# PRBonn/LiDiff

Hardware: NVIDIA H100
Metric: denoising_steps_per_sec_180k_pts_T50 (higher is better)
Workload: dtype fp16x3 split tensor-core MMA, fp32 accumulate (fp32 CUDA cores for the Cin=3 stem), fp64 DPM update

## Files before the change

### lidiff_b200/csrc/spconv_tc.cu

```cuda
#include "common.cuh"
#include <algorithm>
#include <stdlib.h>
#include "tc_common.cuh"

namespace tc {

constexpr int THREADS = 384;
constexpr int NUM_PRODUCER = 128;
constexpr int NUM_CONSUMER_WARPS = 8;
constexpr int STEP_BUDGET = 64;
constexpr int MAX_KVOL = 27;
constexpr int MAX_STAGES = 4;

struct Params {
    int c1, c2, cout, kvol;
    const unsigned char* wpacked;
    const float* scale;
    const float* shift;
    int relu;
    const int* nbr;
    long long nbr_stride;
    const int* d_mout;
    int mout_cap;
    const int* row_perm;
    const unsigned* row_mask;
    const int* tile_order;
    int stages, nchunks, group;
    int npass, nsplit;
    lb2_conv_io io[2];
};

constexpr int PRODUCER_REGS = 88;
constexpr int CONSUMER_REGS = 208;
static_assert(128 * PRODUCER_REGS + 256 * CONSUMER_REGS <= THREADS * 168, "register split exceeds the CTA's allocation");

template <int NC>
__global__ void __launch_bounds__(THREADS, 1) k_spconv_tc(const Params p) {
    extern __shared__ unsigned char smem_raw[];
    const int M = p.d_mout ? min(*p.d_mout, p.mout_cap) : p.mout_cap;
    const int half = blockIdx.x % p.nsplit;
    const int pass = (blockIdx.x / p.nsplit) % p.npass;
    const int slot_i = blockIdx.x / (p.nsplit * p.npass);
    const int tile = p.tile_order ? __ldg(p.tile_order + slot_i) : slot_i;
    const int m0 = tile * BM;
    if (tile < 0 || m0 >= M) return;
    const lb2_conv_io io = p.io[pass];
    const int n0 = half * NC;
    const int warp = threadIdx.x >> 5, lane = threadIdx.x & 31;
    const int ctot = p.c1 + p.c2;

    const uint32_t raw = smem_u32(smem_raw);
    const uint32_t base = (raw + 1023u) & ~1023u;
    unsigned char* gen = smem_raw + (base - raw);
    constexpr uint32_t b_tile = (uint32_t)NC * 128u;
    const uint32_t b_full = (uint32_t)p.cout * 128u;
    const uint32_t stage_bytes = 2u * A_TILE + 2u * b_tile;
    unsigned char* tail = gen + (size_t)p.stages * stage_bytes;
    int* idx_s = reinterpret_cast<int*>(tail);
    uint64_t* bars = reinterpret_cast<uint64_t*>(tail + MAX_KVOL * BM * sizeof(int));
    uint32_t* misc = reinterpret_cast<uint32_t*>(bars + 3 * MAX_STAGES);
    int* row_s = reinterpret_cast<int*>(misc + 4);
    const uint32_t bar0 = smem_u32(bars);
    auto full_a = [&](int s) { return bar0 + 8u * s; };
    auto full_b = [&](int s) { return bar0 + 8u * (MAX_STAGES + s); };
    auto empty = [&](int s) { return bar0 + 8u * (2 * MAX_STAGES + s); };

    if (threadIdx.x == 0) {
        for (int s = 0; s < p.stages; ++s) { mbar_init(full_a(s), NUM_PRODUCER); mbar_init(full_b(s), 1); mbar_init(empty(s), NUM_CONSUMER_WARPS); }
        misc[1] = 0;
        asm volatile("fence.mbarrier_init.release.cluster;" ::: "memory");
    }
    __syncthreads();
    if (threadIdx.x < BM) {
        const int slot = m0 + threadIdx.x;
        const int row = (slot < M) ? (p.row_perm ? __ldg(p.row_perm + slot) : slot) : -1;
        row_s[threadIdx.x] = row;
        const uint32_t want = row < 0 ? 0u : (p.row_mask ? __ldg(p.row_mask + row) : ~0u);
        int v[MAX_KVOL];
#pragma unroll
        for (int k = 0; k < MAX_KVOL; ++k) {
            v[k] = -1;
            if (k < p.kvol && ((want >> k) & 1u)) v[k] = p.nbr ? __ldg(p.nbr + (long long)k * p.nbr_stride + row) : row;
        }
        uint32_t have = 0;
#pragma unroll
        for (int k = 0; k < MAX_KVOL; ++k) {
            if (k < p.kvol) {
                idx_s[k * BM + threadIdx.x] = v[k];
                if (v[k] >= 0) have |= 1u << k;
            }
        }
        const uint32_t mymask = __reduce_or_sync(0xffffffffu, have);
        if (lane == 0 && mymask) atomicOr(&misc[1], mymask);
    }
    __syncthreads();
    const uint32_t kmask = misc[1];
    const int n_off = __popc(kmask);

    if (warpgroup_role() == 0) {
        setmaxnreg_dec<PRODUCER_REGS>();
        const int sub = threadIdx.x & 7;
        const int rbase = threadIdx.x >> 3;
        const bool use_h = (io.in1_h != nullptr) && (p.c2 == 0 || io.in2_h != nullptr);
        const int D = max(p.stages - 2, 0);
        int it = 0, arrived = 0;
        for (uint32_t km = kmask; km; km &= km - 1) {
            const int k = __ffs(km) - 1;
            const int* idxk = idx_s + k * BM;
            int src[8];
#pragma unroll
            for (int j = 0; j < 8; ++j) src[j] = idxk[rbase + 16 * j];
            for (int c = 0; c < p.nchunks; ++c, ++it) {
                const int s = it % p.stages;
                mbar_wait(empty(s), ((it / p.stages) & 1) ^ 1);
                unsigned char* a_hi = gen + (size_t)s * stage_bytes;
                const uint32_t a_hi_u = base + (uint32_t)s * stage_bytes;
                if (threadIdx.x == 0) {
                    const uint32_t dst = a_hi_u + 2u * A_TILE;
                    const unsigned char* wsrc = p.wpacked + PACK_HEADER + ((size_t)k * p.nchunks + c) * (2u * b_full) + (size_t)n0 * 128u;
                    mbar_expect_tx(full_b(s), 2u * b_tile);
                    bulk_g2s(dst, wsrc, b_tile, full_b(s));
                    bulk_g2s(dst + b_tile, wsrc + b_full, b_tile, full_b(s));
                }
                const int ch = c * KC + sub * 8;
                if (ch < ctot) {
                    const bool first = ch < p.c1;
                    const int cw = first ? p.c1 : p.c2;
                    const int co = first ? ch : ch - p.c1;
                    if (use_h) produce_a_split(reinterpret_cast<const __half*>(first ? io.in1_h : io.in2_h), cw, co, src, a_hi_u, a_hi_u + A_TILE, rbase, sub);
                    else produce_a_f32(first ? io.in1 : io.in2, cw, co, src, a_hi, a_hi + A_TILE, rbase, sub);
                }
                if (use_h) {
                    cp_async_commit();
                    if (it >= D) {
                        cp_async_wait_dyn(D);
                        fence_proxy_async();
                        mbar_arrive(full_a(arrived % p.stages));
                        ++arrived;
                    }
                } else {
                    fence_proxy_async();
                    mbar_arrive(full_a(s));
                }
            }
        }
        if (use_h) {
            cp_async_wait<0>();
            fence_proxy_async();
            for (; arrived < it; ++arrived) mbar_arrive(full_a(arrived % p.stages));
        }
    } else {
        setmaxnreg_inc<CONSUMER_REGS>();
        const int wg = (warp >> 2) - 1;
        float acc[NC / 2], tot[NC / 2];
#pragma unroll
        for (int i = 0; i < NC / 2; ++i) tot[i] = -0.f;
        const int n_it = n_off * p.nchunks;
        int c = 0, in_group = 0, off_idx = 0, prev_s = -1;
        for (int it = 0; it < n_it; ++it) {
            const int s = it % p.stages;
            const uint32_t par = (it / p.stages) & 1;
            mbar_wait(full_b(s), par);
            mbar_wait(full_a(s), par);
            const uint32_t a_hi = base + (uint32_t)s * stage_bytes + (uint32_t)wg * (A_TILE / 2), a_lo = a_hi + A_TILE;
            const uint32_t b_hi = base + (uint32_t)s * stage_bytes + 2u * A_TILE, b_lo = b_hi + b_tile;
            const int ksteps = min(KC, ctot - c * KC) >> 4;
            reg_fence(acc);
            wg_stage_mma<NC>(acc, a_hi, a_lo, b_hi, b_lo, ksteps, in_group == 0 && c == 0);
            reg_fence(acc);
            wgmma_wait<1>();
            if (prev_s >= 0 && lane == 0) mbar_arrive(empty(prev_s));
            prev_s = s;
            if (++c < p.nchunks) continue;
            c = 0;
            ++off_idx;
            if (++in_group == p.group || off_idx == n_off) {
                wgmma_wait<0>();
                reg_fence(acc);
                if (lane == 0) mbar_arrive(empty(prev_s));
                prev_s = -1;
#pragma unroll
                for (int i = 0; i < NC / 2; ++i) tot[i] = __fadd_rn(tot[i], acc[i]);
                in_group = 0;
            }
        }
        wgmma_wait<0>();
        const float out_scale = __ldg(reinterpret_cast<const float*>(p.wpacked) + 1);
        float* stage_c = reinterpret_cast<float*>(gen);
        constexpr int pitch = NC + 4;
        asm volatile("bar.sync 1, 256;" ::: "memory");
        {
            const int r0 = wg * 64 + (warp & 3) * 16 + (lane >> 2);
#pragma unroll
            for (int i = 0; i < NC / 2; i += 2) {
                const int row = r0 + 8 * ((i >> 1) & 1), col = 8 * (i >> 2) + 2 * (lane & 3);
                *reinterpret_cast<float2*>(stage_c + row * pitch + col) = make_float2(tot[i] * out_scale, tot[i + 1] * out_scale);
            }
        }
        asm volatile("bar.sync 1, 256;" ::: "memory");
        const int cw = warp - 4;
        constexpr int nv = NC >> 2;
        for (int e = lane; e < (BM / NUM_CONSUMER_WARPS) * nv; e += 32) {
            const int rr = cw + NUM_CONSUMER_WARPS * (e / nv);
            const int lcol = (e % nv) * 4;
            const int col = n0 + lcol;
            const int orow = row_s[rr];
            if (orow < 0) continue;
            const long long ro = (long long)orow * p.cout;
            const float4 a4 = *reinterpret_cast<const float4*>(stage_c + (size_t)rr * pitch + lcol);
            float y[4] = {a4.x, a4.y, a4.z, a4.w};
            if (io.pre_add) {
                const float4 t4 = __ldg(reinterpret_cast<const float4*>(io.pre_add + ro + col));
                y[0] += t4.x; y[1] += t4.y; y[2] += t4.z; y[3] += t4.w;
            }
            if (p.scale) {
                const float4 s4 = __ldg(reinterpret_cast<const float4*>(p.scale + col));
                const float4 h4 = __ldg(reinterpret_cast<const float4*>(p.shift + col));
                y[0] = fmaf(y[0], s4.x, h4.x); y[1] = fmaf(y[1], s4.y, h4.y); y[2] = fmaf(y[2], s4.z, h4.z); y[3] = fmaf(y[3], s4.w, h4.w);
            }
            if (io.residual || io.residual_h) {
                const float4 t4 = load_residual4(io.residual, io.residual_h, orow, p.cout, col);
                y[0] += t4.x; y[1] += t4.y; y[2] += t4.z; y[3] += t4.w;
            }
            if (p.relu) {
#pragma unroll
                for (int j = 0; j < 4; ++j) y[j] = fmaxf(y[j], 0.f);
            }
            if (io.out) *reinterpret_cast<float4*>(io.out + ro + col) = make_float4(y[0], y[1], y[2], y[3]);
            if (io.out_h) store_split4(io.out_h, orow, p.cout, col, y);
            if (io.out_gated || io.out_gated_h) {
                if (io.gate_table) {
                    const long long g = io.gate_idx ? __ldg(io.gate_idx + orow) : 0;
                    const float4 g4 = __ldg(reinterpret_cast<const float4*>(io.gate_table + g * p.cout + col));
                    y[0] *= g4.x; y[1] *= g4.y; y[2] *= g4.z; y[3] *= g4.w;
                }
                if (io.out_gated) *reinterpret_cast<float4*>(io.out_gated + ro + col) = make_float4(y[0], y[1], y[2], y[3]);
                if (io.out_gated_h) store_split4(io.out_gated_h, orow, p.cout, col, y);
            }
        }
    }
}

__global__ void k_weight_absmax(const float* __restrict__ w, long long n, unsigned* __restrict__ header) {
    long long t = (long long)blockIdx.x * blockDim.x + threadIdx.x;
    float m = 0.f;
    for (; t < n; t += (long long)gridDim.x * blockDim.x) m = fmaxf(m, fabsf(w[t]));
#pragma unroll
    for (int o = 16; o > 0; o >>= 1) m = fmaxf(m, __shfl_xor_sync(0xffffffffu, m, o));
    if ((threadIdx.x & 31) == 0) atomicMax(header, __float_as_uint(m));
}

__device__ __forceinline__ float weight_scale(unsigned max_bits) {
    const float m = __uint_as_float(max_bits);
    if (!(m > 0.f) || !isfinite(m)) return 1.f;
    int e;
    frexpf(m, &e);
    return ldexpf(1.f, 14 - e);
}

__global__ void k_pack_weights(const float* __restrict__ w, int kvol, int cin, int cout, int nchunks, unsigned char* __restrict__ out) {
    const long long total = (long long)kvol * nchunks * cout * KC;
    long long t = (long long)blockIdx.x * blockDim.x + threadIdx.x;
    const float scale = weight_scale(*reinterpret_cast<const unsigned*>(out));
    if (t == 0) reinterpret_cast<float*>(out)[1] = 1.0f / scale;
    if (t >= total) return;
    const int kk = (int)(t % KC);
    const int n = (int)((t / KC) % cout);
    const int c = (int)((t / ((long long)KC * cout)) % nchunks);
    const int k = (int)(t / ((long long)KC * cout * nchunks));
    const int ch = c * KC + kk;
    const float v = ch < cin ? w[((long long)k * cin + ch) * cout + n] * scale : 0.f;
    const __half hi = __float2half_rn(v);
    const __half lo = __float2half_rn(v - __half2float(hi));
    const size_t tile = (size_t)cout * 128;
    unsigned char* blob = out + PACK_HEADER + ((size_t)k * nchunks + c) * 2 * tile;
    const uint32_t off = sw128(n, kk >> 3) + (uint32_t)(kk & 7) * 2u;
    *reinterpret_cast<__half*>(blob + off) = hi;
    *reinterpret_cast<__half*>(blob + tile + off) = lo;
}

static bool shape_ok(int c1, int c2, int cout, int kvol) {
    const int ctot = c1 + c2;
    if (kvol < 1 || kvol > MAX_KVOL) return false;
    if (ctot % 16 != 0 || ctot < 16) return false;
    if (c2 > 0 && (c1 % 8 != 0 || c2 % 8 != 0)) return false;
    if (cout % 32 != 0 || cout < 32 || cout > 256) return false;
    if (cout > 128 && cout != 256) return false;
    return true;
}

static size_t smem_bytes(int nc, int stages) {
    return 1024 + (size_t)stages * (2 * A_TILE + 2 * (size_t)nc * 128) + MAX_KVOL * BM * sizeof(int) + 3 * MAX_STAGES * 8 + 16 + BM * sizeof(int);
}

template <int NC>
static int launch(Lb2Handle* h, cudaStream_t s, const Params& p, int stages) {
    const size_t smem = smem_bytes(NC, stages);
    cudaError_t e = lb2_configure_smem(h, LB2_K_TC + (NC / 32 - 1), k_spconv_tc<NC>, (int)(227 * 1024));
    if (e != cudaSuccess) return lb2_fail(h, LB2_ERR_CUDA, "k_spconv_tc smem attribute: %s", cudaGetErrorString(e));
    k_spconv_tc<NC><<<cdiv(p.mout_cap, BM) * p.npass * p.nsplit, THREADS, smem, s>>>(p);
    LB2_POST_LAUNCH(h, "k_spconv_tc");
    return LB2_OK;
}

}

bool lb2_spconv_tc_supported(const lb2_conv_desc* d) { return tc::shape_ok(d->c1, d->c2, d->cout, d->kvol); }

extern "C" size_t lb2_packed_weight_bytes(int32_t kvol, int32_t cin, int32_t cout) {
    if (!tc::shape_ok(cin, 0, cout, kvol)) return 0;
    const int nchunks = (cin + tc::KC - 1) / tc::KC;
    return tc::PACK_HEADER + (size_t)kvol * nchunks * 2 * (size_t)cout * 128;
}

extern "C" int lb2_pack_weights(void* handle, void* stream, const float* weight, int32_t kvol, int32_t cin, int32_t cout, void* packed) {
    Lb2Handle* h = (Lb2Handle*)handle;
    LB2_REQUIRE(h, h && weight && packed, "pack_weights null");
    if (!tc::shape_ok(cin, 0, cout, kvol)) return lb2_fail(h, LB2_ERR_UNSUP, "pack_weights: shape not supported by the tensor-core variant%s", "");
    const int nchunks = (cin + tc::KC - 1) / tc::KC;
    const long long total = (long long)kvol * nchunks * cout * tc::KC;
    const long long nw = (long long)kvol * cin * cout;
    if (cudaMemsetAsync(packed, 0, tc::PACK_HEADER, (cudaStream_t)stream) != cudaSuccess) return lb2_fail(h, LB2_ERR_CUDA, "pack_weights memset%s", "");
    tc::k_weight_absmax<<<(unsigned)std::min<long long>(cdiv(nw, 256), 1024), 256, 0, (cudaStream_t)stream>>>(weight, nw, (unsigned*)packed);
    LB2_POST_LAUNCH(h, "k_weight_absmax");
    tc::k_pack_weights<<<cdiv(total, 256), 256, 0, (cudaStream_t)stream>>>(weight, kvol, cin, cout, nchunks, (unsigned char*)packed);
    LB2_POST_LAUNCH(h, "k_pack_weights");
    return LB2_OK;
}

int lb2_spconv_tc_launch(Lb2Handle* h, cudaStream_t s, const lb2_conv_desc* d) {
    tc::Params p;
    p.c1 = d->c1; p.c2 = d->c2; p.cout = d->cout; p.kvol = d->kvol;
    p.wpacked = (const unsigned char*)d->weight_packed;
    p.scale = d->scale; p.shift = d->shift; p.relu = d->relu;
    p.nbr = d->nbr; p.nbr_stride = d->nbr_stride; p.d_mout = d->d_mout; p.mout_cap = d->mout_cap; p.row_perm = d->row_perm;
    p.tile_order = d->nbr ? d->tile_order128 : nullptr;
    p.row_mask = d->nbr ? (const unsigned*)d->row_mask : nullptr;
    p.nchunks = (d->c1 + d->c2 + tc::KC - 1) / tc::KC;
    const int nsplit = d->cout > 128 ? 2 : 1;
    const int nc = d->cout / nsplit;
    p.npass = d->npass > 1 ? 2 : 1;
    p.nsplit = nsplit;
    int stages = tc::MAX_STAGES;
    while (stages > 2 && tc::smem_bytes(nc, stages) > 227 * 1024) --stages;
    p.stages = stages;
    const int steps_per_offset = 3 * ((d->c1 + d->c2 + 15) / 16);
    p.group = std::max(1, tc::STEP_BUDGET / steps_per_offset);
    p.io[0] = d->io[0]; p.io[1] = d->io[d->npass > 1 ? 1 : 0];
    switch (nc) {
        case 32: return tc::launch<32>(h, s, p, stages);
        case 64: return tc::launch<64>(h, s, p, stages);
        case 96: return tc::launch<96>(h, s, p, stages);
        case 128: return tc::launch<128>(h, s, p, stages);
        default: return lb2_fail(h, LB2_ERR_UNSUP, "tensor-core variant: no kernel for %s output channels per CTA", nc == 80 ? "80" : nc == 112 ? "112" : "this many");
    }
}
```

Baseline: 25.98.

## Make sparse-conv tensor-core kernel persistent with double-buffered tile metadata

Turns the warp-specialized sparse conv kernel into a persistent kernel with a grid capped at the SM count. Each CTA walks tiles in a grid-stride loop. The producer warpgroup prefetches the next tile's neighbor indices into a double-buffered shared TileInfo, and the epilogue staging reuses a pipeline stage buffer with an XOR swizzle instead of a padded pitch. The aim is to remove per-CTA launch and setup costs and to overlap index loading and the epilogue with the next tile's MMA pipeline. In exchange it adds more complex barrier and parity bookkeeping and an extra pipeline slot per tile, and tile_order load balancing becomes a static round-robin.

After: 27.39 (median of 6 runs). 1.05x the previous value.

```diff
diff --git a/lidiff_b200/csrc/spconv_tc.cu b/lidiff_b200/csrc/spconv_tc.cu
--- a/lidiff_b200/csrc/spconv_tc.cu
+++ b/lidiff_b200/csrc/spconv_tc.cu
@@ -34,20 +34,22 @@
 constexpr int CONSUMER_REGS = 208;
 static_assert(128 * PRODUCER_REGS + 256 * CONSUMER_REGS <= THREADS * 168, "register split exceeds the CTA's allocation");
 
+struct TileInfo {
+    int idx[MAX_KVOL * BM];
+    int row[BM];
+    uint32_t mask[4];
+    int item;
+    int pad[3];
+};
+constexpr int NUM_BARS = 3 * MAX_STAGES + 4;
+
 template <int NC>
 __global__ void __launch_bounds__(THREADS, 1) k_spconv_tc(const Params p) {
     extern __shared__ unsigned char smem_raw[];
     const int M = p.d_mout ? min(*p.d_mout, p.mout_cap) : p.mout_cap;
-    const int half = blockIdx.x % p.nsplit;
-    const int pass = (blockIdx.x / p.nsplit) % p.npass;
-    const int slot_i = blockIdx.x / (p.nsplit * p.npass);
-    const int tile = p.tile_order ? __ldg(p.tile_order + slot_i) : slot_i;
-    const int m0 = tile * BM;
-    if (tile < 0 || m0 >= M) return;
-    const lb2_conv_io io = p.io[pass];
-    const int n0 = half * NC;
     const int warp = threadIdx.x >> 5, lane = threadIdx.x & 31;
     const int ctot = p.c1 + p.c2;
+    const int S = p.stages;
 
     const uint32_t raw = smem_u32(smem_raw);
     const uint32_t base = (raw + 1023u) & ~1023u;
@@ -55,187 +57,229 @@
     constexpr uint32_t b_tile = (uint32_t)NC * 128u;
     const uint32_t b_full = (uint32_t)p.cout * 128u;
     const uint32_t stage_bytes = 2u * A_TILE + 2u * b_tile;
-    unsigned char* tail = gen + (size_t)p.stages * stage_bytes;
-    int* idx_s = reinterpret_cast<int*>(tail);
-    uint64_t* bars = reinterpret_cast<uint64_t*>(tail + MAX_KVOL * BM * sizeof(int));
-    uint32_t* misc = reinterpret_cast<uint32_t*>(bars + 3 * MAX_STAGES);
-    int* row_s = reinterpret_cast<int*>(misc + 4);
-    const uint32_t bar0 = smem_u32(bars);
+    TileInfo* info = reinterpret_cast<TileInfo*>(gen + (size_t)S * stage_bytes);
+    const uint32_t bar0 = smem_u32(info + 2);
     auto full_a = [&](int s) { return bar0 + 8u * s; };
     auto full_b = [&](int s) { return bar0 + 8u * (MAX_STAGES + s); };
     auto empty = [&](int s) { return bar0 + 8u * (2 * MAX_STAGES + s); };
+    auto info_full = [&](int b) { return bar0 + 8u * (3 * MAX_STAGES + b); };
+    auto info_empty = [&](int b) { return bar0 + 8u * (3 * MAX_STAGES + 2 + b); };
 
     if (threadIdx.x == 0) {
-        for (int s = 0; s < p.stages; ++s) { mbar_init(full_a(s), NUM_PRODUCER); mbar_init(full_b(s), 1); mbar_init(empty(s), NUM_CONSUMER_WARPS); }
-        misc[1] = 0;
+        for (int s = 0; s < S; ++s) { mbar_init(full_a(s), NUM_PRODUCER); mbar_init(full_b(s), 1); mbar_init(empty(s), NUM_CONSUMER_WARPS); }
+        for (int b = 0; b < 2; ++b) { mbar_init(info_full(b), NUM_PRODUCER); mbar_init(info_empty(b), NUM_CONSUMER_WARPS); }
         asm volatile("fence.mbarrier_init.release.cluster;" ::: "memory");
     }
     __syncthreads();
-    if (threadIdx.x < BM) {
-        const int slot = m0 + threadIdx.x;
-        const int row = (slot < M) ? (p.row_perm ? __ldg(p.row_perm + slot) : slot) : -1;
-        row_s[threadIdx.x] = row;
-        const uint32_t want = row < 0 ? 0u : (p.row_mask ? __ldg(p.row_mask + row) : ~0u);
-        int v[MAX_KVOL];
-#pragma unroll
-        for (int k = 0; k < MAX_KVOL; ++k) {
-            v[k] = -1;
-            if (k < p.kvol && ((want >> k) & 1u)) v[k] = p.nbr ? __ldg(p.nbr + (long long)k * p.nbr_stride + row) : row;
-        }
-        uint32_t have = 0;
-#pragma unroll
-        for (int k = 0; k < MAX_KVOL; ++k) {
-            if (k < p.kvol) {
-                idx_s[k * BM + threadIdx.x] = v[k];
-                if (v[k] >= 0) have |= 1u << k;
-            }
-        }
-        const uint32_t mymask = __reduce_or_sync(0xffffffffu, have);
-        if (lane == 0 && mymask) atomicOr(&misc[1], mymask);
-    }
-    __syncthreads();
-    const uint32_t kmask = misc[1];
-    const int n_off = __popc(kmask);
 
     if (warpgroup_role() == 0) {
         setmaxnreg_dec<PRODUCER_REGS>();
         const int sub = threadIdx.x & 7;
         const int rbase = threadIdx.x >> 3;
-        const bool use_h = (io.in1_h != nullptr) && (p.c2 == 0 || io.in2_h != nullptr);
-        const int D = max(p.stages - 2, 0);
+        const int D = max(S - 2, 0);
         int it = 0, arrived = 0;
-        for (uint32_t km = kmask; km; km &= km - 1) {
-            const int k = __ffs(km) - 1;
-            const int* idxk = idx_s + k * BM;
-            int src[8];
-#pragma unroll
-            for (int j = 0; j < 8; ++j) src[j] = idxk[rbase + 16 * j];
-            for (int c = 0; c < p.nchunks; ++c, ++it) {
-                const int s = it % p.stages;
-                mbar_wait(empty(s), ((it / p.stages) & 1) ^ 1);
-                unsigned char* a_hi = gen + (size_t)s * stage_bytes;
-                const uint32_t a_hi_u = base + (uint32_t)s * stage_bytes;
-                if (threadIdx.x == 0) {
-                    const uint32_t dst = a_hi_u + 2u * A_TILE;
-                    const unsigned char* wsrc = p.wpacked + PACK_HEADER + ((size_t)k * p.nchunks + c) * (2u * b_full) + (size_t)n0 * 128u;
-                    mbar_expect_tx(full_b(s), 2u * b_tile);
-                    bulk_g2s(dst, wsrc, b_tile, full_b(s));
-                    bulk_g2s(dst + b_tile, wsrc + b_full, b_tile, full_b(s));
-                }
-                const int ch = c * KC + sub * 8;
-                if (ch < ctot) {
-                    const bool first = ch < p.c1;
-                    const int cw = first ? p.c1 : p.c2;
-                    const int co = first ? ch : ch - p.c1;
-                    if (use_h) produce_a_split(reinterpret_cast<const __half*>(first ? io.in1_h : io.in2_h), cw, co, src, a_hi_u, a_hi_u + A_TILE, rbase, sub);
-                    else produce_a_f32(first ? io.in1 : io.in2, cw, co, src, a_hi, a_hi + A_TILE, rbase, sub);
-                }
-                if (use_h) {
+        auto tile_of = [&](int x) {
+            const int slot_i = x / (p.nsplit * p.npass);
+            return slot_i * BM >= p.mout_cap ? -1 : p.tile_order ? __ldg(p.tile_order + slot_i) : slot_i;
+        };
+        auto load_row = [&](int tile) {
+            const int slot = tile * BM + threadIdx.x;
+            return (tile >= 0 && slot < M) ? (p.row_perm ? __ldg(p.row_perm + slot) : slot) : -1;
+        };
+        auto load_indices = [&](int row, int (&v)[MAX_KVOL]) {
+            const uint32_t want = row < 0 ? 0u : (p.row_mask ? __ldg(p.row_mask + row) : ~0u);
+#pragma unroll
+            for (int k = 0; k < MAX_KVOL; ++k) {
+                v[k] = -1;
+                if (k < p.kvol && ((want >> k) & 1u)) v[k] = p.nbr ? __ldg(p.nbr + (long long)k * p.nbr_stride + row) : row;
+            }
+        };
+        int x = blockIdx.x, tile = tile_of(x), row = load_row(tile), v[MAX_KVOL];
+        load_indices(row, v);
+        for (int j = 0;; ++j) {
+            TileInfo& ti = info[j & 1];
+            mbar_wait(info_empty(j & 1), ((j >> 1) & 1) ^ 1);
+            if (tile < 0 || tile * BM >= M) {
+                if (threadIdx.x == 0) ti.item = -1;
+                mbar_arrive(info_full(j & 1));
+                break;
+            }
+            {
+                ti.row[threadIdx.x] = row;
+                uint32_t have = 0;
+#pragma unroll
+                for (int k = 0; k < MAX_KVOL; ++k) {
+                    if (k < p.kvol) {
+                        ti.idx[k * BM + threadIdx.x] = v[k];
+                        if (v[k] >= 0) have |= 1u << k;
+                    }
+                }
+                const uint32_t wmask = __reduce_or_sync(0xffffffffu, have);
+                if (lane == 0) ti.mask[warp] = wmask;
+                if (threadIdx.x == 0) ti.item = x;
+            }
+            mbar_arrive(info_full(j & 1));
+            mbar_wait(info_full(j & 1), (j >> 1) & 1);
+            const uint32_t kmask = ti.mask[0] | ti.mask[1] | ti.mask[2] | ti.mask[3];
+            const int x_next = x + gridDim.x;
+            const int tile_next = tile_of(x_next);
+            const int n0 = (x % p.nsplit) * NC;
+            const lb2_conv_io io = p.io[(x / p.nsplit) % p.npass];
+            const bool use_h = (io.in1_h != nullptr) && (p.c2 == 0 || io.in2_h != nullptr);
+            for (uint32_t km = kmask; km; km &= km - 1) {
+                const int k = __ffs(km) - 1;
+                const int* idxk = ti.idx + k * BM;
+                int src[8];
+#pragma unroll
+                for (int r = 0; r < 8; ++r) src[r] = idxk[rbase + 16 * r];
+                for (int c = 0; c < p.nchunks; ++c) {
+                    const int s = it % S;
+                    mbar_wait(empty(s), ((it / S) & 1) ^ 1);
+                    unsigned char* a_hi = gen + (size_t)s * stage_bytes;
+                    const uint32_t a_hi_u = base + (uint32_t)s * stage_bytes;
+                    if (threadIdx.x == 0) {
+                        const uint32_t dst = a_hi_u + 2u * A_TILE;
+                        const unsigned char* wsrc = p.wpacked + PACK_HEADER + ((size_t)k * p.nchunks + c) * (2u * b_full) + (size_t)n0 * 128u;
+                        mbar_expect_tx(full_b(s), 2u * b_tile);
+                        bulk_g2s(dst, wsrc, b_tile, full_b(s));
+                        bulk_g2s(dst + b_tile, wsrc + b_full, b_tile, full_b(s));
+                    }
+                    const int ch = c * KC + sub * 8;
+                    if (ch < ctot) {
+                        const bool first = ch < p.c1;
+                        const int cw = first ? p.c1 : p.c2;
+                        const int co = first ? ch : ch - p.c1;
+                        if (use_h) produce_a_split(reinterpret_cast<const __half*>(first ? io.in1_h : io.in2_h), cw, co, src, a_hi_u, a_hi_u + A_TILE, rbase, sub);
+                        else produce_a_f32(first ? io.in1 : io.in2, cw, co, src, a_hi, a_hi + A_TILE, rbase, sub);
+                    }
                     cp_async_commit();
-                    if (it >= D) {
+                    ++it;
+                    if (it - arrived > D) {
                         cp_async_wait_dyn(D);
                         fence_proxy_async();
-                        mbar_arrive(full_a(arrived % p.stages));
+                        mbar_arrive(full_a(arrived % S));
                         ++arrived;
                     }
-                } else {
-                    fence_proxy_async();
-                    mbar_arrive(full_a(s));
-                }
-            }
-        }
-        if (use_h) {
+                }
+            }
+            const int s = it % S;
+            mbar_wait(empty(s), ((it / S) & 1) ^ 1);
+            if (threadIdx.x == 0) mbar_arrive(full_b(s));
+            ++it;
+            x = x_next;
+            tile = tile_next;
+            row = load_row(tile);
             cp_async_wait<0>();
             fence_proxy_async();
-            for (; arrived < it; ++arrived) mbar_arrive(full_a(arrived % p.stages));
+            for (; arrived < it; ++arrived) mbar_arrive(full_a(arrived % S));
+            load_indices(row, v);
         }
     } else {
         setmaxnreg_inc<CONSUMER_REGS>();
         const int wg = (warp >> 2) - 1;
-        float acc[NC / 2], tot[NC / 2];
-#pragma unroll
-        for (int i = 0; i < NC / 2; ++i) tot[i] = -0.f;
-        const int n_it = n_off * p.nchunks;
-        int c = 0, in_group = 0, off_idx = 0, prev_s = -1;
-        for (int it = 0; it < n_it; ++it) {
-            const int s = it % p.stages;
-            const uint32_t par = (it / p.stages) & 1;
-            mbar_wait(full_b(s), par);
-            mbar_wait(full_a(s), par);
-            const uint32_t a_hi = base + (uint32_t)s * stage_bytes + (uint32_t)wg * (A_TILE / 2), a_lo = a_hi + A_TILE;
-            const uint32_t b_hi = base + (uint32_t)s * stage_bytes + 2u * A_TILE, b_lo = b_hi + b_tile;
-            const int ksteps = min(KC, ctot - c * KC) >> 4;
-            reg_fence(acc);
-            wg_stage_mma<NC>(acc, a_hi, a_lo, b_hi, b_lo, ksteps, in_group == 0 && c == 0);
-            reg_fence(acc);
-            wgmma_wait<1>();
-            if (prev_s >= 0 && lane == 0) mbar_arrive(empty(prev_s));
-            prev_s = s;
-            if (++c < p.nchunks) continue;
-            c = 0;
-            ++off_idx;
-            if (++in_group == p.group || off_idx == n_off) {
-                wgmma_wait<0>();
+        const float out_scale = __ldg(reinterpret_cast<const float*>(p.wpacked) + 1);
+        int it = 0;
+        for (int j = 0;; ++j) {
+            const TileInfo& ti = info[j & 1];
+            mbar_wait(info_full(j & 1), (j >> 1) & 1);
+            const int x = ti.item;
+            if (x < 0) break;
+            const int n_off = __popc(ti.mask[0] | ti.mask[1] | ti.mask[2] | ti.mask[3]);
+            float acc[NC / 2], tot[NC / 2];
+#pragma unroll
+            for (int i = 0; i < NC / 2; ++i) tot[i] = -0.f;
+            const int n_it = n_off * p.nchunks;
+            int c = 0, in_group = 0, off_idx = 0, prev_s = -1;
+            for (int i = 0; i < n_it; ++i, ++it) {
+                const int s = it % S;
+                const uint32_t par = (it / S) & 1;
+                mbar_wait(full_b(s), par);
+                mbar_wait(full_a(s), par);
+                const uint32_t a_hi = base + (uint32_t)s * stage_bytes + (uint32_t)wg * (A_TILE / 2), a_lo = a_hi + A_TILE;
+                const uint32_t b_hi = base + (uint32_t)s * stage_bytes + 2u * A_TILE, b_lo = b_hi + b_tile;
+                const int ksteps = min(KC, ctot - c * KC) >> 4;
                 reg_fence(acc);
-                if (lane == 0) mbar_arrive(empty(prev_s));
-                prev_s = -1;
-#pragma unroll
-                for (int i = 0; i < NC / 2; ++i) tot[i] = __fadd_rn(tot[i], acc[i]);
-                in_group = 0;
-            }
-        }
-        wgmma_wait<0>();
-        const float out_scale = __ldg(reinterpret_cast<const float*>(p.wpacked) + 1);
-        float* stage_c = reinterpret_cast<float*>(gen);
-        constexpr int pitch = NC + 4;
-        asm volatile("bar.sync 1, 256;" ::: "memory");
-        {
-            const int r0 = wg * 64 + (warp & 3) * 16 + (lane >> 2);
-#pragma unroll
-            for (int i = 0; i < NC / 2; i += 2) {
-                const int row = r0 + 8 * ((i >> 1) & 1), col = 8 * (i >> 2) + 2 * (lane & 3);
-                *reinterpret_cast<float2*>(stage_c + row * pitch + col) = make_float2(tot[i] * out_scale, tot[i + 1] * out_scale);
-            }
-        }
-        asm volatile("bar.sync 1, 256;" ::: "memory");
-        const int cw = warp - 4;
-        constexpr int nv = NC >> 2;
-        for (int e = lane; e < (BM / NUM_CONSUMER_WARPS) * nv; e += 32) {
-            const int rr = cw + NUM_CONSUMER_WARPS * (e / nv);
-            const int lcol = (e % nv) * 4;
-            const int col = n0 + lcol;
-            const int orow = row_s[rr];
-            if (orow < 0) continue;
-            const long long ro = (long long)orow * p.cout;
-            const float4 a4 = *reinterpret_cast<const float4*>(stage_c + (size_t)rr * pitch + lcol);
-            float y[4] = {a4.x, a4.y, a4.z, a4.w};
-            if (io.pre_add) {
-                const float4 t4 = __ldg(reinterpret_cast<const float4*>(io.pre_add + ro + col));
-                y[0] += t4.x; y[1] += t4.y; y[2] += t4.z; y[3] += t4.w;
-            }
-            if (p.scale) {
-                const float4 s4 = __ldg(reinterpret_cast<const float4*>(p.scale + col));
-                const float4 h4 = __ldg(reinterpret_cast<const float4*>(p.shift + col));
-                y[0] = fmaf(y[0], s4.x, h4.x); y[1] = fmaf(y[1], s4.y, h4.y); y[2] = fmaf(y[2], s4.z, h4.z); y[3] = fmaf(y[3], s4.w, h4.w);
-            }
-            if (io.residual || io.residual_h) {
-                const float4 t4 = load_residual4(io.residual, io.residual_h, orow, p.cout, col);
-                y[0] += t4.x; y[1] += t4.y; y[2] += t4.z; y[3] += t4.w;
-            }
-            if (p.relu) {
-#pragma unroll
-                for (int j = 0; j < 4; ++j) y[j] = fmaxf(y[j], 0.f);
-            }
-            if (io.out) *reinterpret_cast<float4*>(io.out + ro + col) = make_float4(y[0], y[1], y[2], y[3]);
-            if (io.out_h) store_split4(io.out_h, orow, p.cout, col, y);
-            if (io.out_gated || io.out_gated_h) {
-                if (io.gate_table) {
-                    const long long g = io.gate_idx ? __ldg(io.gate_idx + orow) : 0;
-                    const float4 g4 = __ldg(reinterpret_cast<const float4*>(io.gate_table + g * p.cout + col));
-                    y[0] *= g4.x; y[1] *= g4.y; y[2] *= g4.z; y[3] *= g4.w;
-                }
-                if (io.out_gated) *reinterpret_cast<float4*>(io.out_gated + ro + col) = make_float4(y[0], y[1], y[2], y[3]);
-                if (io.out_gated_h) store_split4(io.out_gated_h, orow, p.cout, col, y);
+                wg_stage_mma<NC>(acc, a_hi, a_lo, b_hi, b_lo, ksteps, in_group == 0 && c == 0);
+                reg_fence(acc);
+                wgmma_wait<1>();
+                if (prev_s >= 0 && lane == 0) mbar_arrive(empty(prev_s));
+                prev_s = s;
+                if (++c < p.nchunks) continue;
+                c = 0;
+                ++off_idx;
+                if (++in_group == p.group || off_idx == n_off) {
+                    wgmma_wait<0>();
+                    reg_fence(acc);
+                    if (lane == 0) mbar_arrive(empty(prev_s));
+                    prev_s = -1;
+#pragma unroll
+                    for (int i = 0; i < NC / 2; ++i) tot[i] = __fadd_rn(tot[i], acc[i]);
+                    in_group = 0;
+                }
+            }
+            wgmma_wait<0>();
+            const int se = it % S;
+            mbar_wait(full_b(se), (it / S) & 1);
+            mbar_wait(full_a(se), (it / S) & 1);
+            ++it;
+            float* stage_c = reinterpret_cast<float*>(gen + (size_t)se * stage_bytes);
+            {
+                const int r0 = wg * 64 + (warp & 3) * 16 + (lane >> 2);
+#pragma unroll
+                for (int i = 0; i < NC / 2; i += 2) {
+                    const int row = r0 + 8 * ((i >> 1) & 1), col = 8 * (i >> 2) + 2 * (lane & 3);
+                    *reinterpret_cast<float2*>(stage_c + row * NC + (((col >> 2) ^ (row & 7)) << 2) + (col & 3)) =
+                        make_float2(tot[i] * out_scale, tot[i + 1] * out_scale);
+                }
+            }
+            asm volatile("bar.sync 1, 256;" ::: "memory");
+            const lb2_conv_io io = p.io[(x / p.nsplit) % p.npass];
+            const int n0 = (x % p.nsplit) * NC;
+            const int cw = warp - 4;
+            constexpr int nv = NC >> 2;
+            for (int e = lane; e < (BM / NUM_CONSUMER_WARPS) * nv; e += 32) {
+                const int rr = cw + NUM_CONSUMER_WARPS * (e / nv);
+                const int lcol = (e % nv) * 4;
+                const int col = n0 + lcol;
+                const int orow = ti.row[rr];
+                if (orow < 0) continue;
+                const long long ro = (long long)orow * p.cout;
+                const float4 a4 = *reinterpret_cast<const float4*>(stage_c + rr * NC + (((lcol >> 2) ^ (rr & 7)) << 2));
+                float y[4] = {a4.x, a4.y, a4.z, a4.w};
+                if (io.pre_add) {
+                    const float4 t4 = __ldg(reinterpret_cast<const float4*>(io.pre_add + ro + col));
+                    y[0] += t4.x; y[1] += t4.y; y[2] += t4.z; y[3] += t4.w;
+                }
+                if (p.scale) {
+                    const float4 s4 = __ldg(reinterpret_cast<const float4*>(p.scale + col));
+                    const float4 h4 = __ldg(reinterpret_cast<const float4*>(p.shift + col));
+                    y[0] = fmaf(y[0], s4.x, h4.x); y[1] = fmaf(y[1], s4.y, h4.y); y[2] = fmaf(y[2], s4.z, h4.z); y[3] = fmaf(y[3], s4.w, h4.w);
+                }
+                if (io.residual || io.residual_h) {
+                    const float4 t4 = load_residual4(io.residual, io.residual_h, orow, p.cout, col);
+                    y[0] += t4.x; y[1] += t4.y; y[2] += t4.z; y[3] += t4.w;
+                }
+                if (p.relu) {
+#pragma unroll
+                    for (int q = 0; q < 4; ++q) y[q] = fmaxf(y[q], 0.f);
+                }
+                if (io.out) *reinterpret_cast<float4*>(io.out + ro + col) = make_float4(y[0], y[1], y[2], y[3]);
+                if (io.out_h) store_split4(io.out_h, orow, p.cout, col, y);
+                if (io.out_gated || io.out_gated_h) {
+                    if (io.gate_table) {
+                        const long long g = io.gate_idx ? __ldg(io.gate_idx + orow) : 0;
+                        const float4 g4 = __ldg(reinterpret_cast<const float4*>(io.gate_table + g * p.cout + col));
+                        y[0] *= g4.x; y[1] *= g4.y; y[2] *= g4.z; y[3] *= g4.w;
+                    }
+                    if (io.out_gated) *reinterpret_cast<float4*>(io.out_gated + ro + col) = make_float4(y[0], y[1], y[2], y[3]);
+                    if (io.out_gated_h) store_split4(io.out_gated_h, orow, p.cout, col, y);
+                }
+            }
+            fence_proxy_async();
+            __syncwarp();
+            if (lane == 0) {
+                mbar_arrive(empty(se));
+                mbar_arrive(info_empty(j & 1));
             }
         }
     }
@@ -290,7 +334,7 @@
 }
 
 static size_t smem_bytes(int nc, int stages) {
-    return 1024 + (size_t)stages * (2 * A_TILE + 2 * (size_t)nc * 128) + MAX_KVOL * BM * sizeof(int) + 3 * MAX_STAGES * 8 + 16 + BM * sizeof(int);
+    return 1024 + (size_t)stages * (2 * A_TILE + 2 * (size_t)nc * 128) + 2 * sizeof(TileInfo) + NUM_BARS * sizeof(uint64_t);
 }
 
 template <int NC>
@@ -298,7 +342,8 @@
     const size_t smem = smem_bytes(NC, stages);
     cudaError_t e = lb2_configure_smem(h, LB2_K_TC + (NC / 32 - 1), k_spconv_tc<NC>, (int)(227 * 1024));
     if (e != cudaSuccess) return lb2_fail(h, LB2_ERR_CUDA, "k_spconv_tc smem attribute: %s", cudaGetErrorString(e));
-    k_spconv_tc<NC><<<cdiv(p.mout_cap, BM) * p.npass * p.nsplit, THREADS, smem, s>>>(p);
+    const unsigned grid = (unsigned)std::min<long long>(h->num_sms, (long long)cdiv(p.mout_cap, BM) * p.npass * p.nsplit);
+    k_spconv_tc<NC><<<grid, THREADS, smem, s>>>(p);
     LB2_POST_LAUNCH(h, "k_spconv_tc");
     return LB2_OK;
 }
```
